# torchmd/torchmd-net

Measured on AMD Instinct MI355X. Metric: molecules/sec (64-atom molecules) TensorNet E+F, higher is better.
Workload: dtype f32; 1 GPU; BASELINE configs[1]: TensorNet F=128 L=2 K=32 rc=5.0, S-mol64 256 molecules x 64 atoms per GPU, energies + forces, random-init weights (seed 0); atoms_per_gpu=16384, pairs_per_gpu=193709, directed_edges_per_gpu=403802, parallelism=molecule-sharded x1, RCCL all-reduce of energies, rank_step=eager: tmdnet_build_graph (pair-count read-back) + tmdnet_energy_forces

## Files before the change

### torchmd-net_amd/csrc/tn_api.hip

```cpp
#include <hip/hip_runtime.h>

#include <algorithm>
#include <cmath>
#include <cstdio>
#include <cstdlib>
#include <cstring>
#include <map>
#include <unordered_map>
#include <string>
#include <vector>

#include "tn_chain.h"
#include "tn_heads.h"
#include "tn_model.h"
#include "tn_tlin9.h"
#include "tn_small.h"
#include "tn_interp.h"
#include "tn_virial.h"

using namespace tn;

static const char* kCatNames[CAT_COUNT] = {"graph", "gemm_edge", "gemm_node", "message", "pair_bwd", "embed_scatter", "elementwise", "edge_table"};

int fail(tmdnet_model* m, int code, const std::string& msg) {
// ... 448 lines not shown
    out.err_slope = worst_s;
    if (getenv("TMDNET_DEBUG"))
      fprintf(stderr, "[tmdnet] radial tables T=%d: value err %.3e, slope err %.3e, fail=%d\n", T, worst_v, worst_s, (int)fail_);
    cleanup(good);
    if (good) {
      out.ok = true;
      out.T = T;
      out.tab = tab;
      for (const TableSpec& sp : specs) out.R.push_back(sp.chain.back().N);
      return TMDNET_OK;
    }
    if (fail_) return TMDNET_OK;
  }
  (void)m;
  return TMDNET_OK;
}

namespace {

int build_edge_tables(tmdnet_model* m) {
  const tmdnet_hparams& hp = m->hp;
  const int F = hp.hidden_channels, K = hp.num_rbf, L = hp.num_layers;
  const DevParams& W = m->P;
  std::vector<TableSpec> specs;
  if (m->tn2) {
    specs.push_back(TableSpec{{TableLayer{W.Wdp, W.bdp, 3 * F, K, 0}}});
    for (int l = 0; l < L; ++l) specs.push_back(TableSpec{{TableLayer{m->tn2->layer[l].M1a, W.layer[l].b1, F, K, 0}}});
  } else if (L + 1 <= 8) {
    specs.push_back(TableSpec{{TableLayer{W.Wdp, W.bdp, 3 * F, K, 0}}});
    for (int l = 0; l < L; ++l) {
      const LayerP& q_ = W.layer[l];
      specs.push_back(TableSpec{{TableLayer{q_.M1, q_.b1, F, K, 1}, TableLayer{q_.M2, q_.b2, 2 * F, F, 1},
                                 TableLayer{q_.M3, q_.b3, 3 * F, 2 * F, 2}}});
    }
  }
  return build_radial_tables(m, m->tabs, specs, W.means, W.betas, K, hp.cutoff_lower, hp.cutoff_upper);
}

}

int ensure_radial_tables(tmdnet_model* m, hipStream_t s) {
  if (!m->tabs_pending) return TMDNET_OK;
  hipStreamCaptureStatus cs = hipStreamCaptureStatusNone;
  if (s && hipStreamIsCapturing(s, &cs) == hipSuccess && cs != hipStreamCaptureStatusNone)
    return fail(m, TMDNET_ERR_STATE, "the radial tables are rebuilt after a parameter upload: run one step outside the capture first");
  HIP_TRY(m, hipDeviceSynchronize());
  const int rc = m->et ? et_build_tables(m) : build_edge_tables(m);
  if (rc != TMDNET_OK) return rc;
  HIP_TRY(m, hipStreamSynchronize(nullptr));
  m->tabs_pending = false;
  return TMDNET_OK;
}

extern "C" {

const char* tmdnet_version(void) { return "tmdnet_amd 0.3 (gfx950)"; }
int tmdnet_abi_version(void) { return TMDNET_ABI_VERSION; }

int tmdnet_create(const tmdnet_hparams* hp, tmdnet_model** out) {
  if (!hp || !out) return TMDNET_ERR_INVALID;
  if (hp->hidden_channels <= 0 || hp->num_layers < 0 || hp->num_rbf <= 0 || hp->max_z <= 0 || hp->head_hidden <= 0 ||
      hp->max_num_neighbors <= 0 || !(hp->cutoff_upper > hp->cutoff_lower))
    return TMDNET_ERR_INVALID;
  tmdnet_model* m = new tmdnet_model();
  m->hp = *hp;
  if (const char* e = getenv("TMDNET_EDGE_TABLE_MIN_PAIRS")) m->tab_min_pairs = atoll(e);
  build_specs(m);
  if (getenv("TMDNET_SIDE_STREAM")) {
    if (hipStreamCreateWithFlags(&m->side, hipStreamNonBlocking) != hipSuccess) m->side = nullptr;
    if (m->side) {
      (void)hipEventCreateWithFlags(&m->ev_fork, hipEventDisableTiming);
      m->ev_join.resize(hp->num_layers);
      for (auto& e : m->ev_join) (void)hipEventCreateWithFlags(&e, hipEventDisableTiming);
    }
  }
  *out = m;
  return TMDNET_OK;
}

int tmdnet_create_tn2(const tmdnet_tn2_hparams* hp, tmdnet_model** out) {
  if (!hp || !out) return TMDNET_ERR_INVALID;
  if (hp->hidden_channels <= 0 || hp->num_layers < 0 || hp->num_rbf <= 0 || hp->max_z <= 0 || hp->head_hidden <= 0 ||
      hp->max_num_neighbors <= 0 || !(hp->cutoff_upper > hp->cutoff_lower) || hp->q_dim <= 0 || hp->q_dim > 64 ||
      (hp->num_layers + 1) * hp->q_dim > 64)
    return TMDNET_ERR_INVALID;
  tmdnet_model* m = new tmdnet_model();
  m->hp = tmdnet_hparams{hp->hidden_channels, hp->num_layers, hp->num_rbf, hp->max_z, hp->max_num_neighbors, hp->group_o3,
                         hp->head_hidden, hp->has_atomref, hp->cutoff_lower, hp->cutoff_upper};
  m->tn2 = new Tn2Model();
  m->tn2->hp = *hp;
  if (const char* e = getenv("TMDNET_EDGE_TABLE_MIN_PAIRS")) m->tab_min_pairs = atoll(e);
  build_specs(m);
  *out = m;
  return TMDNET_OK;
}

int tmdnet_create_et(const tmdnet_et_hparams* hp, tmdnet_model** out) {
  if (!hp || !out) return TMDNET_ERR_INVALID;
  if (hp->hidden_channels <= 0 || hp->num_layers < 0 || hp->num_rbf <= 0 || hp->max_z <= 0 || hp->num_heads <= 0 ||
      hp->max_num_neighbors <= 0 || !(hp->cutoff_upper > hp->cutoff_lower))
    return TMDNET_ERR_INVALID;
  tmdnet_model* m = new tmdnet_model();
  m->hp = tmdnet_hparams{};
  m->hp.hidden_channels = hp->hidden_channels;
  m->hp.num_layers = hp->num_layers;
  m->hp.num_rbf = hp->num_rbf;
  m->hp.max_z = hp->max_z;
  m->hp.max_num_neighbors = hp->max_num_neighbors;
  m->hp.has_atomref = hp->has_atomref;
  m->hp.cutoff_lower = hp->cutoff_lower;
  m->hp.cutoff_upper = hp->cutoff_upper;
  const int rc = et_create(m, hp);
  if (rc != TMDNET_OK) {
    delete m;
    return rc;
  }
  *out = m;
  return TMDNET_OK;
}

int tmdnet_destroy(tmdnet_model* m) {
  if (!m) return TMDNET_OK;
  et_destroy(m);
  if (m->side) {
    (void)hipStreamSynchronize(m->side);
    (void)hipEventDestroy(m->ev_fork);
    for (auto& e : m->ev_join) (void)hipEventDestroy(e);
    (void)hipStreamDestroy(m->side);
  }
  free_radial_tables(m->tabs);
  delete m->tn2;
  if (m->dev) (void)hipFree(m->dev);
  if (m->dev_sb) (void)hipFree(m->dev_sb);
  if (m->upd_tid) (void)hipFree(m->upd_tid);
  if (m->upd_ofs) (void)hipFree(m->upd_ofs);
  if (m->upd_ptrs) (void)hipFree(m->upd_ptrs);
  if (m->rb_img) (void)hipFree(m->rb_img);
  if (m->halo_rng) (void)hipFree(m->halo_rng);
  if (m->prior_tab) (void)hipFree(m->prior_tab);
  delete m;
  return TMDNET_OK;
}

const char* tmdnet_last_error(const tmdnet_model* m) { return m ? m->err.c_str() : "null model"; }

int tmdnet_num_params(const tmdnet_model* m) { return m ? (int)m->specs.size() : 0; }

int tmdnet_set_output_head(tmdnet_model* m, int32_t kind) {
  if (!m) return TMDNET_ERR_INVALID;
  if (kind < TMDNET_HEAD_SCALAR || kind > TMDNET_HEAD_VECTOR)
    return fail(m, TMDNET_ERR_INVALID, "unknown output head kind " + std::to_string(kind));
  if (kind != TMDNET_HEAD_SCALAR && m->tn2)
    return fail(m, TMDNET_ERR_INVALID, "TensorNet2 has the ScalarPlusWeightedCoulomb head only (no property heads)");
  if (kind == TMDNET_HEAD_VECTOR && !m->et)
    return fail(m, TMDNET_ERR_INVALID, "the vector output head needs the Equivariant Transformer's vector features");
  m->host.clear();
  m->finalized = false;
  m->upd_ready = false;
  m->head_kind = kind;
  if (m->et) {
    et_head_specs(m);
    return TMDNET_OK;
  }
  const std::string key = "output_model.atomic_mass";
  auto& sp = m->specs;
  for (size_t i = 0; i < sp.size(); ++i)
    if (sp[i].name == key) {
      sp.erase(sp.begin() + (long)i);
      break;
    }
  if (kind != TMDNET_HEAD_SCALAR) sp.push_back({key, TMDNET_MASS_TABLE_SIZE, 1});
  return TMDNET_OK;
}

const char* tmdnet_param_name(const tmdnet_model* m, int idx, int64_t* numel) {
  if (!m || idx < 0 || idx >= (int)m->specs.size()) return nullptr;
  if (numel) *numel = m->specs[idx].rows * m->specs[idx].cols;
  return m->specs[idx].name.c_str();
}

int tmdnet_set_param(tmdnet_model* m, const char* name, const float* data_host, int64_t numel) {
  if (!m || !name || !data_host) return TMDNET_ERR_INVALID;
  for (const auto& sp : m->specs) {
    if (sp.name == name) {
      if (numel != sp.rows * sp.cols)
        return fail(m, TMDNET_ERR_INVALID, std::string("parameter ") + name + ": expected " + std::to_string(sp.rows * sp.cols) +
                                               " elements, got " + std::to_string(numel));
      m->host[name].assign(data_host, data_host + numel);
      m->finalized = false;
      return TMDNET_OK;
    }
// ... 470 lines not shown
    if (const int rc = ensure_radial_tables(const_cast<tmdnet_model*>(m), nullptr)) return rc;
  if (n == "edge_table_T") *value = m->tabs.ok ? m->tabs.T : 0;
  else if (n == "edge_table_err_value") *value = m->tabs.err_value;
  else if (n == "edge_table_err_slope") *value = m->tabs.err_slope;
  else if (n == "edge_table_min_pairs") *value = (double)m->tab_min_pairs;
  else if (n == "pair_rows_bf16") *value = (double)m->pair_bf16;
  else if (n == "embed_rb_min_atoms") *value = (double)m->rb_min_atoms;
  else if (n == "chain_min_atoms") *value = (double)m->chain_min_atoms;
  else if (n == "chain_mask") *value = (double)m->chain_mask;
  else if (n == "chain_last") *value = (double)m->chain_last;
  else if (n == "recompute_pair_rows") *value = m->recompute_rows ? 1.0 : 0.0;
  else if (n == "embed_rb") *value = m->rb_fwd ? 1.0 : 0.0;
  else if (n == "species_last_build") *value = (double)m->last_nt;
  else if (n == "halo_active_first") *value = (double)m->halo_active[0];
  else if (n == "halo_active_rows") *value = (double)m->halo_active[1];
  else if (n == "message_route_last") *value = (double)m->msg_route_last[0];
  else if (n == "message_adjoint_route_last") *value = (double)m->msg_route_last[1];
  else if (n == "fold_node_adjoint") *value = m->fold_node_adjoint ? 1.0 : 0.0;
  else if (n == "message_adjoint_fold_last") *value = (double)m->msg_fold_last;
  else return TMDNET_ERR_INVALID;
  return TMDNET_OK;
}

int tmdnet_set_cell_grid(tmdnet_model* m, int32_t ncx, int32_t ncy, int32_t ncz) {
  if (!m) return TMDNET_ERR_INVALID;
  if (ncx < 0 || ncy < 0 || ncz < 0) ncx = ncy = ncz = -1;
  m->cell_n[0] = ncx;
  m->cell_n[1] = ncy;
  m->cell_n[2] = ncz;
  return TMDNET_OK;
}

int tmdnet_graph_workspace_bytes(const tmdnet_model* m, int64_t n_atoms, int64_t n_mol, size_t* bytes) {
  if (!m || !bytes || n_atoms < 0 || n_mol < 0) return TMDNET_ERR_INVALID;
  const int64_t ecap = (int64_t)m->hp.max_num_neighbors * n_atoms;
  carve_graph(nullptr, n_atoms, n_mol, ecap, bytes);
  return TMDNET_OK;
}

int tmdnet_build_graph(tmdnet_model* m, void* stream, void* graph_ws, size_t graph_ws_bytes, int64_t n_atoms, int64_t n_mol,
                       const float* pos, const int64_t* batch, const int64_t* z, const float* box, int32_t box_mode,
                       int64_t counts_host[8]) {
  if (!m || !graph_ws || !counts_host || n_atoms < 0 || n_mol < 0) return TMDNET_ERR_INVALID;
  if (n_atoms >= (int64_t)1 << 30) return fail(m, TMDNET_ERR_INVALID, "n_atoms too large for 32-bit indices");
  hipStream_t s = reinterpret_cast<hipStream_t>(stream);
  const int64_t ecap = (int64_t)m->hp.max_num_neighbors * n_atoms;
  size_t need = 0;
  Graph g = carve_graph(graph_ws, n_atoms, n_mol, ecap, &need);
  if (need > graph_ws_bytes) return fail(m, TMDNET_ERR_WORKSPACE, "graph workspace too small");
  if (box_mode != 0 && !box) return fail(m, TMDNET_ERR_INVALID, "box_mode != 0 needs a box");
  const bool cell = cell_applicable(m, n_atoms, n_mol, box_mode);
  set_cell(g, m, cell, n_mol);
  if (cell && m->halo_fn && m->atom_w && !m->et && !m->tn2) g.ghost_w = m->atom_w;
  m->graph_no_ghost_pairs = g.ghost_w != nullptr;
  m->graph_is_cell = cell;
  m->graph_cell_multi = cell && n_mol > 1;
  m->graph_has_z = z != nullptr;
  m->g_pos = pos;
  m->g_box = box;
  m->g_box_mode = box_mode;
  CurScope cur_(m);
  {
    ProfScope ps_(s, CAT_GRAPH, 0.0, (double)n_atoms * 20);
    if (cell) {
      launch_fill(reinterpret_cast<float*>(g.counts), 0.f, 8, s);
      launch_cell_phase1(g, pos, batch, box_mode == 1 ? box : nullptr, (int)n_atoms, m->hp.cutoff_lower, m->hp.cutoff_upper, true, s,
                         (int)n_mol);
      launch_scan_counts(g, (int)n_atoms, s);
    } else {
      launch_graph_build_phase1(g, pos, batch, box, box_mode, (int)n_atoms, (int)n_mol, m->hp.cutoff_lower, m->hp.cutoff_upper,
                                true, s);
    }
    if (z) launch_prepare_z(g, z, cell ? g.perm : nullptr, (int)n_atoms, m->hp.max_z, s);
    if (z && m->rb_fwd && n_atoms >= m->rb_min_atoms) launch_type_map(g, (int)n_atoms, m->hp.max_z, s);
  }
  int counts[8] = {0, 0, 0, 0, 0, 0, 0, 0};
  HIP_TRY(m, hipMemcpyAsync(counts, g.counts, sizeof(counts), hipMemcpyDeviceToHost, s));
  HIP_TRY(m, hipStreamSynchronize(s));
  for (int k = 0; k < 8; ++k) counts_host[k] = counts[k];
  m->last_nt = (z && m->rb_fwd && n_atoms >= m->rb_min_atoms) ? counts[6] : 0;
  m->lastE = counts[1];
  m->graph_closed_tiles = !cell && counts[3] == 0 && counts[5] == 0 && counts[7] == 0;
  remember_graph(m, graph_ws, n_atoms, n_mol);
  if (counts[5])
    return fail(m, TMDNET_ERR_INVALID, "batch index out of range: every entry must be in [0, " + std::to_string(n_mol) + ")");
  if (counts[4])
    return fail(m, TMDNET_ERR_INVALID, "atomic number out of range: every z must be in [0, max_z = " + std::to_string(m->hp.max_z) + ")");
  if (counts[2])
    return fail(m, TMDNET_ERR_OVERFLOW, "Found num_pairs > max_num_pairs, please increase max_num_pairs (found " +
                                            std::to_string(counts[1]) + " edges, capacity " + std::to_string(ecap) + ")");
  m->lastE = counts[1];
  {
    ProfScope ps_(s, CAT_GRAPH, 0.0, (double)counts[1] * 12 + (double)counts[0] * 40);
    if (cell) {
      launch_cell_phase2(g, (int)n_atoms, m->hp.cutoff_lower, m->hp.cutoff_upper, true, s);
      launch_nbr_link_wave(g, (int)n_atoms, s);
    } else {
      launch_graph_build_phase2(g, pos, batch, box, box_mode, (int)n_atoms, (int)n_mol, m->hp.cutoff_lower, m->hp.cutoff_upper, true,
                                s);
    }
  }
  HIP_TRY(m, hipGetLastError());
  return TMDNET_OK;
}

int tmdnet_build_graph_static(tmdnet_model* m, void* stream, void* graph_ws, size_t graph_ws_bytes, int64_t n_atoms, int64_t n_mol,
                              const float* pos, const int64_t* batch, const int64_t* z, const float* box, int32_t box_mode) {
  if (!m || !graph_ws || n_atoms < 0 || n_mol < 0) return TMDNET_ERR_INVALID;
  hipStream_t s = reinterpret_cast<hipStream_t>(stream);
  const int64_t ecap = (int64_t)m->hp.max_num_neighbors * n_atoms;
  size_t need = 0;
  Graph g = carve_graph(graph_ws, n_atoms, n_mol, ecap, &need);
  if (need > graph_ws_bytes) return fail(m, TMDNET_ERR_WORKSPACE, "graph workspace too small");
  if (box_mode != 0 && !box) return fail(m, TMDNET_ERR_INVALID, "box_mode != 0 needs a box");
  const bool cell = cell_applicable(m, n_atoms, n_mol, box_mode);
  set_cell(g, m, cell, n_mol);
  m->graph_no_ghost_pairs = false;
  m->graph_is_cell = cell;
  m->graph_cell_multi = cell && n_mol > 1;
  m->graph_has_z = z != nullptr;
  m->g_pos = pos;
  m->g_box = box;
  m->g_box_mode = box_mode;
  CurScope cur_(m);
  {
    ProfScope ps_(s, CAT_GRAPH, 0.0, (double)n_atoms * 20);
    if (cell) {
      launch_fill(reinterpret_cast<float*>(g.counts), 0.f, 8, s);
      launch_cell_phase1(g, pos, batch, box_mode == 1 ? box : nullptr, (int)n_atoms, m->hp.cutoff_lower, m->hp.cutoff_upper, true, s,
                         (int)n_mol);
      launch_scan_counts(g, (int)n_atoms, s);
      launch_cell_phase2(g, (int)n_atoms, m->hp.cutoff_lower, m->hp.cutoff_upper, true, s);
      launch_nbr_link_wave(g, (int)n_atoms, s);
    } else if (graph_small_ok((int)n_atoms)) {
      launch_graph_small(g, pos, batch, box, box_mode, (int)n_atoms, (int)n_mol, m->hp.cutoff_lower, m->hp.cutoff_upper, true, z,
                         m->hp.max_z, s);
    } else {
      launch_graph_build_phase1(g, pos, batch, box, box_mode, (int)n_atoms, (int)n_mol, m->hp.cutoff_lower, m->hp.cutoff_upper,
                                true, s);
      launch_graph_build_phase2(g, pos, batch, box, box_mode, (int)n_atoms, (int)n_mol, m->hp.cutoff_lower, m->hp.cutoff_upper, true,
                                s);
    }
    if (z && (cell || !graph_small_ok((int)n_atoms))) launch_prepare_z(g, z, cell ? g.perm : nullptr, (int)n_atoms, m->hp.max_z, s);
  }
  m->lastE = ecap;
  m->last_nt = 0;
  m->graph_closed_tiles = false;
  remember_graph(m, graph_ws, n_atoms, n_mol);
  HIP_TRY(m, hipGetLastError());
  return TMDNET_OK;
}

int tmdnet_graph_counts(tmdnet_model* m, void* stream, void* graph_ws, int64_t n_atoms, int64_t n_mol, int64_t counts_host[8]) {
  if (!m || !graph_ws || !counts_host) return TMDNET_ERR_INVALID;
// ... 1154 lines not shown
```

### torchmd-net_amd/csrc/tn_cell.hip

```cpp
#include <cstring>

#include <hip/hip_runtime.h>

#include "tn_common.h"
#include "tn_kernels.h"

namespace tn {

static inline int cdivc(int64_t a, int64_t b) { return (int)((a + b - 1) / b); }

size_t cell_sort_temp_bytes(int64_t n) { return (size_t)(8 * (n > 0 ? n : 1) + 2) * sizeof(int); }

__global__ void k_cell_assign(const float* __restrict__ pos, const float* __restrict__ box, int N, const int* __restrict__ cgrid,
                              int* __restrict__ key, int* __restrict__ hist) {
  int i = blockIdx.x * blockDim.x + threadIdx.x;
  if (i >= N) return;
  const int ncx = cgrid[0], ncy = cgrid[1], ncz = cgrid[2];
  const float x = pos[i * 3], y = pos[i * 3 + 1], zc = pos[i * 3 + 2];
  float fz = zc / box[8];
  float fy = (y - fz * box[7]) / box[4];
  float fx = (x - fy * box[3] - fz * box[6]) / box[0];
  fx -= floorf(fx);
  fy -= floorf(fy);
  fz -= floorf(fz);
// ... 71 lines not shown
__global__ void k_permute_pos(const float* __restrict__ pos, const int64_t* __restrict__ batch, const int* __restrict__ perm, int N,
                              int B, float* __restrict__ pos_s, int* __restrict__ bat_s, int64_t* __restrict__ bat_c,
                              int* __restrict__ counts) {
  int i = blockIdx.x * blockDim.x + threadIdx.x;
  if (i >= N) return;
  const int o = perm[i];
  pos_s[i * 3] = pos[o * 3];
  pos_s[i * 3 + 1] = pos[o * 3 + 1];
  pos_s[i * 3 + 2] = pos[o * 3 + 2];
  if (batch) {
    int64_t b = batch[o];
    if (B > 0 && (b < 0 || b >= B)) {
      counts[5] = 1;
      b = b < 0 ? 0 : B - 1;
    }
    bat_s[i] = (int)b;
    bat_c[i] = b;
    if (i == 0) counts[3] = 1;
  }
}
__global__ void k_permute_z(const int64_t* __restrict__ z, const int* __restrict__ perm, int N, int64_t* __restrict__ z_s) {
  int i = blockIdx.x * blockDim.x + threadIdx.x;
  if (i < N) z_s[i] = z[perm[i]];
}
void launch_permute_z(const Graph& g, const int64_t* z, int N, hipStream_t s) {
  hipLaunchKernelGGL(k_permute_z, dim3(cdivc(N, 256)), dim3(256), 0, s, z, g.perm, N, g.z_s);
}
__global__ void k_prepare_z(const int64_t* __restrict__ z, const int* __restrict__ perm, int N, int max_z, int64_t* __restrict__ z_c,
                            int* __restrict__ counts) {
  int i = blockIdx.x * blockDim.x + threadIdx.x;
  if (i >= N) return;
  int64_t v = z[perm ? perm[i] : i];
  if (v < 0 || v >= max_z) {
    counts[4] = 1;
    v = v < 0 ? 0 : max_z - 1;
  }
  z_c[i] = v;
}
void launch_prepare_z(const Graph& g, const int64_t* z, const int* perm, int N, int max_z, hipStream_t s) {
  if (N <= 0) return;
  hipLaunchKernelGGL(k_prepare_z, dim3(cdivc(N, 256)), dim3(256), 0, s, z, perm, N, max_z, g.z_c, g.counts);
}

__device__ __forceinline__ float cell_d2(const float* __restrict__ pos, int hi, int lo, const float* __restrict__ box, float& dx,
                                         float& dy, float& dz) {
  return pair_geometry(pos, hi, lo, box, dx, dy, dz);
}

template <bool FILL>
__global__ __launch_bounds__(256) void k_nbr_cell(Graph g, int N, float lo2, float up2, int loop) {
  const int i = blockIdx.x * 4 + (threadIdx.x >> 6);
  const int lane = threadIdx.x & 63;
  if (i >= N) return;
  if (FILL && g.counts[2]) return;
  const float* __restrict__ pos = g.pos_s;
  const float* __restrict__ box = g.boxd;
  const int* __restrict__ bat = g.use_cell > 1 ? g.bat_s : nullptr;
  const int ncx = g.cgrid[0], ncy = g.cgrid[1], ncz = g.cgrid[2];
  const int ci = g.cell_key_sorted[i];
  const int bi = bat ? bat[i] : 0;
  const float* __restrict__ gw = g.ghost_w;
  const bool ghost_i = gw && gw[g.perm[i]] == 0.f;
  const int cz = ci % ncz, cy = (ci / ncz) % ncy, cx = ci / (ncz * ncy);
  int nid = 0x7fffffff;
  if (lane < 27) {
    const int dx = lane / 9 - 1, dy = (lane / 3) % 3 - 1, dz = lane % 3 - 1;
    const int x = (cx + dx + ncx) % ncx, y = (cy + dy + ncy) % ncy, zc = (cz + dz + ncz) % ncz;
    nid = (x * ncy + y) * ncz + zc;
  }
#pragma unroll
  for (int k = 2; k <= 32; k <<= 1)
#pragma unroll
    for (int j = k >> 1; j > 0; j >>= 1) {
      const int other = __shfl_xor(nid, j, 64);
      const bool up = ((lane & k) == 0);
      const bool lower = ((lane & j) == 0);
      nid = (lower == up) ? min(nid, other) : max(nid, other);
    }
  const int P = FILL ? g.counts[0] : 0;
  int e = FILL ? g.rowptr[i] : 0, p = FILL ? g.pairptr[i] : 0;
  int nl = 0, nt = 0;
  const unsigned long long lt = lane == 0 ? 0ull : (~0ull >> (64 - lane));
  int t = 0;
  while (t < 27) {
    int c0 = __shfl(nid, t, 64), c1 = c0;
    ++t;
    while (t < 27) {
      const int cn = __shfl(nid, t, 64);
      if (cn != c1 && cn != c1 + 1) break;
      c1 = cn;
      ++t;
    }
    const int j0 = g.cell_start[c0], j1 = g.cell_start[c1 + 1];
    for (int base = j0; base < j1; base += 64) {
      const int j = base + lane;
      bool hit = false, self = false;
      float dx = 0.f, dy = 0.f, dz = 0.f, d2 = 0.f;
      if (j < j1) {
        if (j == i) {
          hit = loop != 0;
          self = true;
        } else if ((!bat || bat[j] == bi) && !(ghost_i && gw[g.perm[j]] == 0.f)) {
          d2 = (j < i) ? cell_d2(pos, i, j, box, dx, dy, dz) : cell_d2(pos, j, i, box, dx, dy, dz);
          hit = d2 < up2 && d2 >= lo2;
        }
      }
      const unsigned long long mall = __ballot(hit);
// ... 127 lines not shown
```

### torchmd-net_amd/csrc/tn_graph_wave.hip

```cpp
#include <cstdlib>

#include "tn_common.h"
#include "tn_kernels.h"

namespace tn {

static inline int cdivw(int64_t a, int64_t b) { return (int)((a + b - 1) / b); }

__device__ __forceinline__ float pair_d2(const float* __restrict__ pos, int hi, int lo, const float* __restrict__ box, float& dx,
                                         float& dy, float& dz) {
  return pair_geometry(pos, hi, lo, box, dx, dy, dz);
}

template <bool FILL>
__device__ __forceinline__ void nbr_wave_row(const Graph& g, const float* __restrict__ pos, const int64_t* __restrict__ batch,
                                             const float* __restrict__ box, int box_mode, int N, int B, float lo2, float up2, int loop,
                                             int i, int lane) {
  int64_t b = batch[i];
  int j0 = 0, j1 = N;
  if (b < 0 || b >= B) {
    b = 0;
    j1 = 0;
  } else if (!g.counts[3]) {
    j0 = g.mstart[b];
// ... 13 lines not shown
        hit = loop != 0;
        self = true;
      } else if (batch[j] == b) {
        d2 = (j < i) ? pair_d2(pos, i, j, bx, dx, dy, dz) : pair_d2(pos, j, i, bx, dx, dy, dz);
        hit = d2 < up2 && d2 >= lo2;
      }
    }
    const unsigned long long mall = __ballot(hit);
    const unsigned long long mlow = __ballot(hit && j < i);
    if (FILL) {
      if (hit) {
        const int ee = e + __popcll(mall & lt);
        g.col[ee] = j;
        if (self) {
          g.epair[ee] = P;
          g.esign[ee] = 0.f;
        } else if (j < i) {
          const int pp = p + __popcll(mlow & lt);
          const float d = sqrtf(d2);
          const float inv = d > 0.f ? 1.0f / d : 0.f;
          g.pair_i[pp] = i;
          g.pair_j[pp] = j;
          g.pd[pp] = d;
          g.pdelta[pp * 3 + 0] = dx; g.pdelta[pp * 3 + 1] = dy; g.pdelta[pp * 3 + 2] = dz;
          g.prhat[pp * 3 + 0] = dx * inv; g.prhat[pp * 3 + 1] = dy * inv; g.prhat[pp * 3 + 2] = dz * inv;
          g.epair[ee] = pp;
          g.esign[ee] = 1.f;
        } else {
          g.epair[ee] = -1;
          g.esign[ee] = -1.f;
        }
      }
      e += __popcll(mall);
      p += __popcll(mlow);
    } else {
      nt += __popcll(mall);
      nl += __popcll(mlow);
    }
  }
  if (!FILL && lane == 0) {
    g.nlow[i] = nl;
    g.ntot[i] = nt;
  }
  if (FILL && i == 0 && lane == 0) g.pd[P] = 0.f;
}

template <bool FILL>
__global__ __launch_bounds__(256) void k_nbr_wave(Graph g, const float* __restrict__ pos, const int64_t* __restrict__ batch,
                                                  const float* __restrict__ box, int box_mode, int N, int B, float lo2, float up2,
                                                  int loop) {
  const int i = blockIdx.x * 4 + (threadIdx.x >> 6);
  const int lane = threadIdx.x & 63;
  if (i >= N) return;
  if (FILL && g.counts[2]) return;
  nbr_wave_row<FILL>(g, pos, batch, box, box_mode, N, B, lo2, up2, loop, i, lane);
}

__device__ __forceinline__ void nbr_link_row(const Graph& g, int i, int lane) {
  const int e0 = g.rowptr[i], e1 = g.rowptr[i + 1];
  for (int e = e0 + lane; e < e1; e += 64) {
    const int j = g.col[e];
    if (j <= i) continue;
    int lo = g.rowptr[j], hi = lo + g.nlow[j] - 1;
    const int base = lo;
    while (lo < hi) {
      const int mid = (lo + hi) >> 1;
      if (g.col[mid] < i) lo = mid + 1; else hi = mid;
    }
    g.epair[e] = g.pairptr[j] + (lo - base);
  }
}
__global__ __launch_bounds__(256) void k_nbr_link_wave(Graph g, int N) {
  const int i = blockIdx.x * 4 + (threadIdx.x >> 6);
  const int lane = threadIdx.x & 63;
  if (i >= N || g.counts[2]) return;
  nbr_link_row(g, i, lane);
}

constexpr int GS_MAX_ATOMS = 256;
constexpr int GS_ECAP = 16384;
__global__ __launch_bounds__(1024) void k_graph_small(Graph g, const float* __restrict__ pos, const int64_t* __restrict__ batch,
                                                      const float* __restrict__ box, int box_mode, int N, int B, float lo2, float up2,
                                                      int loop, const int64_t* __restrict__ z, int max_z) {
  __shared__ int s_mstart[GS_MAX_ATOMS], s_mend[GS_MAX_ATOMS], s_nlow[GS_MAX_ATOMS], s_ntot[GS_MAX_ATOMS];
  __shared__ int s_rowptr[GS_MAX_ATOMS + 1], s_pairptr[GS_MAX_ATOMS + 1], s_counts[8], c_low[4], c_tot[4];
  __shared__ float s_pos[3 * GS_MAX_ATOMS];
  __shared__ int64_t s_batch[GS_MAX_ATOMS];
  __shared__ int s_col[GS_ECAP];
  const bool col_lds = g.ecap <= GS_ECAP;
  const int tid = threadIdx.x, lane = tid & 63, wave = tid >> 6;
  const bool mol_lds = B <= GS_MAX_ATOMS;
  Graph gl = g;
  gl.nlow = s_nlow;
  gl.ntot = s_ntot;
  gl.rowptr = s_rowptr;
  gl.pairptr = s_pairptr;
  gl.counts = s_counts;
  if (mol_lds) {
    gl.mstart = s_mstart;
    gl.mend = s_mend;
  }
  if (col_lds) gl.col = s_col;
  for (int k = tid; k < 3 * N; k += 1024) s_pos[k] = pos[k];
  if (tid < N) s_batch[tid] = batch[tid];
  for (int i = tid; i < B; i += 1024) gl.mstart[i] = gl.mend[i] = 0;
  if (tid < 8) s_counts[tid] = 0;
  __syncthreads();
  if (tid < N) {
    const int i = tid;
    const int64_t b = s_batch[i];
    if (b < 0 || b >= B) {
      s_counts[3] = 1;
      s_counts[5] = 1;
    } else {
      if (i > 0) {
        const int64_t bp = s_batch[i - 1];
        if (bp > b) s_counts[3] = 1;
        if (bp != b) gl.mstart[b] = i;
        else if ((i & 63) == 0) s_counts[7] = 1;
      } else {
        gl.mstart[b] = 0;
      }
      if (i == N - 1 || s_batch[i + 1] != b) gl.mend[b] = i + 1;
    }
    if (z) {
      int64_t v = z[i];
      if (v < 0 || v >= max_z) {
        s_counts[4] = 1;
// ... 97 lines not shown
```

### torchmd-net_amd/csrc/tn_kernels.h

```cpp
#pragma once
#include <hip/hip_runtime.h>
#include <stdint.h>

namespace tn {

struct Graph {
  int* mstart;
  int* mend;
  int* nlow;
  int* ntot;
  int* rowptr;
  int* pairptr;
  int* col;
  int* epair;
  float* esign;
  int* pair_i;
  int* pair_j;
  float* pd;
  float* pdelta;
  float* prhat;
  int* counts;
  int* tix;
  int* tz;
  int64_t ecap, pcap;
  int* perm;
  int* iota;
  int* cell_key;
  int* cell_key_sorted;
  int* cell_start;
  float* pos_s;
  int64_t* z_s;
  float* boxd;
  int* cgrid;
  int* bat_s;
  int64_t* bat_c;
  int64_t* z_c;
  void* sort_tmp;
  size_t sort_tmp_bytes;
  int ncx, ncy, ncz;
  int use_cell;
  const float* ghost_w;
  int max_z;
  int small_mols;
};

struct RadialParams {
  const float* means;
  const float* betas;
  int K;
  float lo, up;
};

void launch_graph_build_phase1(const Graph& g, const float* pos, const int64_t* batch, const float* box, int box_mode, int N,
                               int B, float lo, float up, bool loop, hipStream_t s);
void launch_graph_build_phase2(const Graph& g, const float* pos, const int64_t* batch, const float* box, int box_mode, int N,
                               int B, float lo, float up, bool loop, hipStream_t s);
void launch_export_pairs(const Graph& g, int N, bool include_transpose, bool loop, int64_t max_pairs, const int* perm,
                         int64_t* neighbors, float* deltas, float* distances, int* num_pairs, hipStream_t s);

void launch_neighbor_grad(const int64_t* nb, const float* deltas, const float* dist, const float* g_delta, const float* g_dist,
                          int64_t M, int N, float* out, hipStream_t s);

void launch_radial(const Graph& g, int P, RadialParams rp, float* phi, float* dphi, float* C, float* dC, hipStream_t s);

void launch_ztables(const float* emb, const float* WaT, const float* WbT, const float* b2, int Z, int F, float* Utab, float* Vtab,
                    hipStream_t s);
void launch_embed_scatter(const Graph& g, int N, int F, const int64_t* z, const float* Utab, const float* Vtab, const float* Q,
                          const float* C, float* u0, float* s0n, hipStream_t s);
void launch_layernorm_fwd(const float* x, const float* w, const float* b, int rows, int R, float* y, float* xhat, float* rstd,
                          hipStream_t s);
void launch_layernorm_bwd(const float* g, const float* xhat, const float* rstd, const float* w, int rows, int R, float* gx,
                          hipStream_t s);
void launch_norm_x(const float* X, float* Xh, int N, int F, hipStream_t s);
struct PairRowTable;
enum MsgRoute {
  MSG_NONE = 0,
  MSG_FWD_ROW = 1,
  MSG_FWD_SPLIT = 2,
  MSG_FWD_TILE = 3,
  MSG_ADJ_ROW = 4,
  MSG_ADJ_SPLIT = 5,
  MSG_GD_ROW = 6,
  MSG_GD_SPLIT = 7,
  MSG_GD_TILE = 8,
  MSG_DUAL = 9,
  MSG_DUAL_ACC = 10,
  MSG_FWD_ROW_TABLE = 11,
  MSG_FWD_ROW_RANGE = 12,
  MSG_GD_ROW_TABLE = 13,
  MSG_GD_ROW_OWNED = 14,
  MSG_GD_ROW_TWO = 15,
  MSG_DUAL_SPLIT3 = 16,
};
MsgRoute message_route(const Graph& g, int N, int F, bool rows_from_table = false, int row0 = 0, int nrows = -1);
MsgRoute message_adjoint_route(int N, int F);
MsgRoute message_adjoint_gd_route(const Graph& g, int N, int F, bool rows_from_table = false, int own0 = 0, int own1 = -1,
// ... 127 lines not shown
```

### torchmd-net_amd/csrc/tn_kernels.hip

```cpp
#include "tn_kernels.h"
#include "tn_interp.h"

#include <cstdlib>

#include "tn_common.h"

namespace tn {

static inline int fthreads(int F) {
  int t = ((F + 63) / 64) * 64;
  return t > 256 ? 256 : t;
}
static inline int cdiv(int64_t a, int64_t b) { return (int)((a + b - 1) / b); }

__global__ void k_mol_ranges(const int64_t* __restrict__ batch, int N, int B, int* mstart, int* mend, int* counts) {
  int i = blockIdx.x * blockDim.x + threadIdx.x;
  if (i >= N) return;
  int64_t b = batch[i];
  if (b < 0 || b >= B) {
    counts[3] = 1;
    counts[5] = 1;
    return;
  }
  if (i > 0) {
// ... 78 lines not shown
    for (int off = 1; off < 64; off <<= 1) {
      int ta = __shfl_up(ia, off, 64), tb = __shfl_up(ib, off, 64);
      if (lane >= off) {
        ia += ta;
        ib += tb;
      }
    }
    if (lane == 63) {
      wsum[0][wave] = ia;
      wsum[1][wave] = ib;
    }
    __syncthreads();
    int oa = carry[0] + ia - a, ob = carry[1] + ib - b;
    for (int w = 0; w < wave; ++w) {
      oa += wsum[0][w];
      ob += wsum[1][w];
    }
#pragma unroll
    for (int r = 0; r < PER; ++r) {
      la[tid * PER + r] = oa;
      lb[tid * PER + r] = ob;
      oa += va[r];
      ob += vb[r];
    }
    __syncthreads();
    if (tid == 1023) {
      carry[0] = oa;
      carry[1] = ob;
    }
#pragma unroll
    for (int r = 0; r < PER; ++r) {
      const int i = base + r * 1024 + tid;
      if (i < N) {
        g.pairptr[i] = la[r * 1024 + tid];
        g.rowptr[i] = lb[r * 1024 + tid];
      }
    }
    __syncthreads();
  }
  if (tid == 0) {
    const int P = carry[0], E = carry[1];
    g.pairptr[N] = P;
    g.rowptr[N] = E;
    g.counts[0] = P;
    g.counts[1] = E;
    g.counts[2] = (E > g.ecap || P > g.pcap || g.counts[5]) ? 1 : 0;
  }
}

__global__ void k_nbr_fill(Graph g, const float* __restrict__ pos, const int64_t* __restrict__ batch, const float* __restrict__ box,
                           int box_mode, int N, float lo2, float up2, int loop) {
  int i = blockIdx.x * blockDim.x + threadIdx.x;
  if (i >= N) return;
  if (g.counts[2]) return;
  const int P = g.counts[0];
  int64_t b = batch[i];
  int j0, j1;
  cand_range(g.mstart, g.mend, g.counts, b, N, j0, j1);
  const float* bx = box_mode == 0 ? nullptr : (box_mode == 1 ? box : box + b * 9);
  int e = g.rowptr[i];
  int p = g.pairptr[i];
  for (int j = j0; j < j1; ++j) {
    if (j == i) {
      if (loop) {
        g.col[e] = i;
        g.epair[e] = P;
        g.esign[e] = 0.f;
        ++e;
      }
      continue;
    }
    if (batch[j] != b) continue;
    float dx, dy, dz;
    float d2 = (j < i) ? pair_delta(pos, i, j, bx, dx, dy, dz) : pair_delta(pos, j, i, bx, dx, dy, dz);
    if (d2 < up2 && d2 >= lo2) {
      g.col[e] = j;
      if (j < i) {
        float d = sqrtf(d2);
        float inv = d > 0.f ? 1.0f / d : 0.f;
        g.pair_i[p] = i;
        g.pair_j[p] = j;
        g.pd[p] = d;
        g.pdelta[p * 3 + 0] = dx;
        g.pdelta[p * 3 + 1] = dy;
        g.pdelta[p * 3 + 2] = dz;
        g.prhat[p * 3 + 0] = dx * inv;
        g.prhat[p * 3 + 1] = dy * inv;
        g.prhat[p * 3 + 2] = dz * inv;
        g.epair[e] = p;
        g.esign[e] = 1.f;
        ++p;
      } else {
        g.epair[e] = -1;
        g.esign[e] = -1.f;
      }
      ++e;
    }
  }
  if (i == 0) g.pd[P] = 0.f;
}

__global__ void k_nbr_link(Graph g, int N) {
  int i = blockIdx.x * blockDim.x + threadIdx.x;
  if (i >= N) return;
  if (g.counts[2]) return;
  int e0 = g.rowptr[i], e1 = g.rowptr[i + 1];
  for (int e = e0; e < e1; ++e) {
    int j = g.col[e];
    if (j <= i) continue;
    int lo = g.rowptr[j], hi = lo + g.nlow[j] - 1, base = lo;
    while (lo < hi) {
      int mid = (lo + hi) >> 1;
      if (g.col[mid] < i) lo = mid + 1; else hi = mid;
    }
    g.epair[e] = g.pairptr[j] + (lo - base);
  }
}

__global__ void k_graph_reset(Graph g, int B) {
  const int i = blockIdx.x * blockDim.x + threadIdx.x;
  if (i < B) g.mstart[i] = g.mend[i] = 0;
  if (i < 8) g.counts[i] = 0;
}

void launch_graph_build_phase1(const Graph& g, const float* pos, const int64_t* batch, const float* box, int box_mode, int N,
                               int B, float lo, float up, bool loop, hipStream_t s) {
  hipLaunchKernelGGL(k_graph_reset, dim3(cdiv(B > 8 ? B : 8, 256)), dim3(256), 0, s, g, B);
  if (N <= 0) return;
  hipLaunchKernelGGL(k_mol_ranges, dim3(cdiv(N, 256)), dim3(256), 0, s, batch, N, B, g.mstart, g.mend, g.counts);
  if (getenv("TMDNET_SCALAR_GRAPH"))
    hipLaunchKernelGGL(k_nbr_count, dim3(cdiv(N, 64)), dim3(64), 0, s, g, pos, batch, box, box_mode, N, lo * lo, up * up, (int)loop);
  else
    launch_nbr_count_wave(g, pos, batch, box, box_mode, N, B, lo, up, loop, s);
  hipLaunchKernelGGL(k_scan_counts, dim3(1), dim3(1024), 0, s, g, N);
}

void launch_scan_counts(const Graph& g, int N, hipStream_t s) {
  hipLaunchKernelGGL(k_scan_counts, dim3(1), dim3(1024), 0, s, g, N);
}

void launch_graph_build_phase2(const Graph& g, const float* pos, const int64_t* batch, const float* box, int box_mode, int N,
                               int B, float lo, float up, bool loop, hipStream_t s) {
  if (N <= 0) return;
  if (getenv("TMDNET_SCALAR_GRAPH")) {
    hipLaunchKernelGGL(k_nbr_fill, dim3(cdiv(N, 64)), dim3(64), 0, s, g, pos, batch, box, box_mode, N, lo * lo, up * up, (int)loop);
    hipLaunchKernelGGL(k_nbr_link, dim3(cdiv(N, 64)), dim3(64), 0, s, g, N);
  } else {
    launch_nbr_fill_link_wave(g, pos, batch, box, box_mode, N, B, lo, up, loop, s);
  }
}

__global__ void k_export_pairs(Graph g, int N, int include_transpose, int loop, int64_t max_pairs, const int* __restrict__ perm,
                               int64_t* neighbors, float* deltas, float* distances, int* num_pairs) {
  const int P = g.counts[0];
  const int64_t total = (int64_t)P * (include_transpose ? 2 : 1) + (loop ? N : 0);
  int64_t idx = (int64_t)blockIdx.x * blockDim.x + threadIdx.x;
  if (idx == 0) num_pairs[0] = (int)total;
  if (idx >= max_pairs) return;
// ... 1319 lines not shown
```

### torchmd-net_amd/csrc/tn_model.h

```cpp
#pragma once
#include <hip/hip_runtime.h>

#include <cstdio>
#include <cstring>
#include <map>
#include <string>
#include <unordered_map>
#include <vector>

#include "../../include/tmdnet_amd.h"
#include "tn_gemm.h"
#include "tn_kernels.h"
#include "tn_prior_math.h"
#include "tn_train.h"

using namespace tn;


struct LayerP {
  const float *M1, *b1, *M2, *b2, *M3, *b3;
  const float *M2T, *M3T;
  const float* V[6];
  const float* VT[6];
  const uint16_t* M_sb[3];
// ... 89 lines not shown
  std::vector<Tn2LayerP> layer;
  const float* qweights = nullptr;
};

struct EdgeTables {
  bool ok = false;
  int T = 0;
  std::vector<float*> tab;
  std::vector<int> R;
  double err_value = 0.0, err_slope = 0.0;
};
struct TableLayer {
  const float* W;
  const float* b;
  int N, K, kind;
};
struct TableSpec {
  std::vector<TableLayer> chain;
};

struct TrainCtx {
  int phase = 0;
  const float* gE = nullptr;
  float* grads = nullptr;
  std::map<std::string, int64_t> off;
  std::vector<float*> pre1, he1, pre2, he2, pre3, Ch, Xh;
  float *g3 = nullptr, *g2 = nullptr, *g1 = nullptr;
  float *self_gw = nullptr, *gq = nullptr, *selfq = nullptr, *gZu = nullptr, *gZv = nullptr, *onehot = nullptr, *head = nullptr;
  float *part = nullptr, *wT = nullptr, *forces = nullptr;
  float* at(const std::string& k) const { return grads + off.at(k); }
};

struct tmdnet_model {
  bool recompute_rows = false;
  const float* atom_w = nullptr;
  int (*halo_fn)(void*, int32_t, float*, int64_t, int64_t, const int32_t*, void*) = nullptr;
  void* halo_user = nullptr;
  int* halo_rng = nullptr;
  bool graph_no_ghost_pairs = false;
  int halo_active[2] = {0, 0};
  bool fold_node_adjoint = true;
  bool graph_closed_tiles = false;
  int msg_fold_last = 0;
  int msg_route_last[2] = {0, 0};
  tmdnet_hparams hp;
  int head_kind = 0;
  TrainCtx* train = nullptr;
  float* virial_out = nullptr;
  void* virial_ws = nullptr;
  std::vector<std::pair<std::string, int64_t>> train_entries;
  hipStream_t side = nullptr;
  hipEvent_t ev_fork = nullptr;
  std::vector<hipEvent_t> ev_join;
  EtModel* et = nullptr;
  Tn2Model* tn2 = nullptr;
  const float* g_pos = nullptr;
  const float* g_box = nullptr;
  int g_box_mode = 0;
  Profiler prof;
  int64_t lastE = 0;
  int cell_n[3] = {0, 0, 0};
  bool graph_is_cell = false;
  bool graph_cell_multi = false;
  bool graph_has_z = false;
  struct GraphRecord { bool is_cell, cell_multi, has_z; int nt; int64_t lastE; bool no_ghost_pairs; int64_t n_atoms, n_mol; bool closed_tiles; };
  std::unordered_map<const void*, GraphRecord> graph_rec;
  std::vector<ParamSpec> specs;
  std::map<std::string, std::vector<float>> host;
  float* dev = nullptr;
  size_t dev_cap = 0, dev_sb_cap = 0, rb_cap = 0;
  uint16_t* dev_sb = nullptr;
  std::unordered_map<const float*, const uint16_t*> sb_of;
  std::unordered_map<const float*, const uint16_t*> fm_of;
  struct ImageJob { size_t src_off; int64_t n, k; size_t dst_off; int fm; };
  std::vector<ImageJob> image_jobs;
  size_t packed_elems = 0;
  int32_t* upd_tid = nullptr;
  int32_t* upd_ofs = nullptr;
  const float** upd_ptrs = nullptr;
  bool upd_ready = false;
  DevParams P;
  EdgeTables tabs;
  uint16_t* rb_img = nullptr;
  const uint16_t *rb_fwd = nullptr, *rb_rev = nullptr;
  int last_nt = 0;
  int64_t rb_min_atoms = 1024;
  int64_t chain_min_atoms = 4096;
  int chain_mask = 7;
  int chain_last = 0;
  int pair_bf16 = 0;
  bool tabs_pending = false;
  int64_t tab_min_pairs = 1;
  bool finalized = false;
  std::string err;
  FwdBuffers last{};
  int64_t lastN = 0, lastP = 0;
  bool has_last = false;
  const float* tn2_last_chg = nullptr;
  int prior_flags = 0, prior_max_z = 0;
  float* prior_tab = nullptr;
  size_t prior_cap = 0;
  tn_prior::ZblConst prior_zbl{};
  tn_prior::D2Const prior_d2{};
};


// ... 97 lines not shown
```

Before: 116,500 molecules/s.

## Overlap graph phase-2 build with pinned pair-count read-back

The pair counts are now read back into a pinned host buffer with an event, and the phase-2 neighbour fill/link kernels are queued before the host waits, so the copy and the host sync overlap with the GPU's fill work instead of leaving the device idle. Because phase 2 now runs before the host checks overflow, the kernels gain a device-side guard (refuse_z with counts[4]) so they skip writing when an error flag is set. This removes a host round-trip bubble per step. The risk is that error handling now depends on device-side flags rather than host checks made before launch.

Result: no change. 117,500 molecules/s (median of 6 runs) (+0.9%).

```diff
diff --git a/torchmd-net_amd/csrc/tn_api.hip b/torchmd-net_amd/csrc/tn_api.hip
--- a/torchmd-net_amd/csrc/tn_api.hip
+++ b/torchmd-net_amd/csrc/tn_api.hip
@@ -524,6 +524,27 @@
   return TMDNET_OK;
 }
 
+static int ensure_counts_readback(tmdnet_model* m) {
+  if (!m->counts_pin) {
+    void* p = nullptr;
+    if (hipHostMalloc(&p, 8 * sizeof(int), hipHostMallocDefault) != hipSuccess) {
+      (void)hipGetLastError();
+      return fail(m, TMDNET_ERR_HIP, "hipHostMalloc of the graph counts' read-back buffer failed");
+    }
+    m->counts_pin = static_cast<int*>(p);
+  }
+  if (!m->ev_counts && hipEventCreateWithFlags(&m->ev_counts, hipEventDisableTiming) != hipSuccess) {
+    (void)hipGetLastError();
+    m->ev_counts = nullptr;
+    return fail(m, TMDNET_ERR_HIP, "hipEventCreate of the graph counts' read-back event failed");
+  }
+  return TMDNET_OK;
+}
+static void create_counts_readback(tmdnet_model* m) {
+  (void)ensure_counts_readback(m);
+  m->err.clear();
+}
+
 extern "C" {
 
 const char* tmdnet_version(void) { return "tmdnet_amd 0.3 (gfx950)"; }
@@ -546,6 +567,7 @@
       for (auto& e : m->ev_join) (void)hipEventCreateWithFlags(&e, hipEventDisableTiming);
     }
   }
+  create_counts_readback(m);
   *out = m;
   return TMDNET_OK;
 }
@@ -563,6 +585,7 @@
   m->tn2->hp = *hp;
   if (const char* e = getenv("TMDNET_EDGE_TABLE_MIN_PAIRS")) m->tab_min_pairs = atoll(e);
   build_specs(m);
+  create_counts_readback(m);
   *out = m;
   return TMDNET_OK;
 }
@@ -587,6 +610,7 @@
     delete m;
     return rc;
   }
+  create_counts_readback(m);
   *out = m;
   return TMDNET_OK;
 }
@@ -609,6 +633,8 @@
   if (m->upd_ptrs) (void)hipFree(m->upd_ptrs);
   if (m->rb_img) (void)hipFree(m->rb_img);
   if (m->halo_rng) (void)hipFree(m->halo_rng);
+  if (m->ev_counts) (void)hipEventDestroy(m->ev_counts);
+  if (m->counts_pin) (void)hipHostFree(m->counts_pin);
   if (m->prior_tab) (void)hipFree(m->prior_tab);
   delete m;
   return TMDNET_OK;
@@ -1185,6 +1211,7 @@
   const bool cell = cell_applicable(m, n_atoms, n_mol, box_mode);
   set_cell(g, m, cell, n_mol);
   if (cell && m->halo_fn && m->atom_w && !m->et && !m->tn2) g.ghost_w = m->atom_w;
+  g.refuse_z = 1;
   m->graph_no_ghost_pairs = g.ghost_w != nullptr;
   m->graph_is_cell = cell;
   m->graph_cell_multi = cell && n_mol > 1;
@@ -1207,10 +1234,24 @@
     if (z) launch_prepare_z(g, z, cell ? g.perm : nullptr, (int)n_atoms, m->hp.max_z, s);
     if (z && m->rb_fwd && n_atoms >= m->rb_min_atoms) launch_type_map(g, (int)n_atoms, m->hp.max_z, s);
   }
-  int counts[8] = {0, 0, 0, 0, 0, 0, 0, 0};
-  HIP_TRY(m, hipMemcpyAsync(counts, g.counts, sizeof(counts), hipMemcpyDeviceToHost, s));
-  HIP_TRY(m, hipStreamSynchronize(s));
-  for (int k = 0; k < 8; ++k) counts_host[k] = counts[k];
+  if (const int rc = ensure_counts_readback(m)) return rc;
+  HIP_TRY(m, hipMemcpyAsync(m->counts_pin, g.counts, 8 * sizeof(int), hipMemcpyDeviceToHost, s));
+  HIP_TRY(m, hipEventRecord(m->ev_counts, s));
+  int ps2 = -1;
+  {
+    ProfScope ps_(s, CAT_GRAPH, 0.0, 0.0);
+    ps2 = ps_.idx;
+    if (cell) {
+      launch_cell_phase2(g, (int)n_atoms, m->hp.cutoff_lower, m->hp.cutoff_upper, true, s);
+      launch_nbr_link_wave(g, (int)n_atoms, s);
+    } else {
+      launch_graph_build_phase2(g, pos, batch, box, box_mode, (int)n_atoms, (int)n_mol, m->hp.cutoff_lower, m->hp.cutoff_upper, true,
+                                s);
+    }
+  }
+  HIP_TRY(m, hipEventSynchronize(m->ev_counts));
+  int counts[8];
+  for (int k = 0; k < 8; ++k) counts_host[k] = counts[k] = m->counts_pin[k];
   m->last_nt = (z && m->rb_fwd && n_atoms >= m->rb_min_atoms) ? counts[6] : 0;
   m->lastE = counts[1];
   m->graph_closed_tiles = !cell && counts[3] == 0 && counts[5] == 0 && counts[7] == 0;
@@ -1223,16 +1264,7 @@
     return fail(m, TMDNET_ERR_OVERFLOW, "Found num_pairs > max_num_pairs, please increase max_num_pairs (found " +
                                             std::to_string(counts[1]) + " edges, capacity " + std::to_string(ecap) + ")");
   m->lastE = counts[1];
-  {
-    ProfScope ps_(s, CAT_GRAPH, 0.0, (double)counts[1] * 12 + (double)counts[0] * 40);
-    if (cell) {
-      launch_cell_phase2(g, (int)n_atoms, m->hp.cutoff_lower, m->hp.cutoff_upper, true, s);
-      launch_nbr_link_wave(g, (int)n_atoms, s);
-    } else {
-      launch_graph_build_phase2(g, pos, batch, box, box_mode, (int)n_atoms, (int)n_mol, m->hp.cutoff_lower, m->hp.cutoff_upper, true,
-                                s);
-    }
-  }
+  if (ps2 >= 0) m->prof.recs[ps2].bytes = (double)counts[1] * 12 + (double)counts[0] * 40;
   HIP_TRY(m, hipGetLastError());
   return TMDNET_OK;
 }
diff --git a/torchmd-net_amd/csrc/tn_cell.hip b/torchmd-net_amd/csrc/tn_cell.hip
--- a/torchmd-net_amd/csrc/tn_cell.hip
+++ b/torchmd-net_amd/csrc/tn_cell.hip
@@ -147,7 +147,7 @@
   const int i = blockIdx.x * 4 + (threadIdx.x >> 6);
   const int lane = threadIdx.x & 63;
   if (i >= N) return;
-  if (FILL && g.counts[2]) return;
+  if (FILL && (g.counts[2] || (g.refuse_z && g.counts[4]))) return;
   const float* __restrict__ pos = g.pos_s;
   const float* __restrict__ box = g.boxd;
   const int* __restrict__ bat = g.use_cell > 1 ? g.bat_s : nullptr;
diff --git a/torchmd-net_amd/csrc/tn_graph_wave.hip b/torchmd-net_amd/csrc/tn_graph_wave.hip
--- a/torchmd-net_amd/csrc/tn_graph_wave.hip
+++ b/torchmd-net_amd/csrc/tn_graph_wave.hip
@@ -89,7 +89,7 @@
   const int i = blockIdx.x * 4 + (threadIdx.x >> 6);
   const int lane = threadIdx.x & 63;
   if (i >= N) return;
-  if (FILL && g.counts[2]) return;
+  if (FILL && (g.counts[2] || (g.refuse_z && g.counts[4]))) return;
   nbr_wave_row<FILL>(g, pos, batch, box, box_mode, N, B, lo2, up2, loop, i, lane);
 }
 
@@ -110,7 +110,7 @@
 __global__ __launch_bounds__(256) void k_nbr_link_wave(Graph g, int N) {
   const int i = blockIdx.x * 4 + (threadIdx.x >> 6);
   const int lane = threadIdx.x & 63;
-  if (i >= N || g.counts[2]) return;
+  if (i >= N || (g.counts[2] || (g.refuse_z && g.counts[4]))) return;
   nbr_link_row(g, i, lane);
 }
 
diff --git a/torchmd-net_amd/csrc/tn_kernels.h b/torchmd-net_amd/csrc/tn_kernels.h
--- a/torchmd-net_amd/csrc/tn_kernels.h
+++ b/torchmd-net_amd/csrc/tn_kernels.h
@@ -42,6 +42,7 @@
   const float* ghost_w;
   int max_z;
   int small_mols;
+  int refuse_z;
 };
 
 struct RadialParams {
diff --git a/torchmd-net_amd/csrc/tn_kernels.hip b/torchmd-net_amd/csrc/tn_kernels.hip
--- a/torchmd-net_amd/csrc/tn_kernels.hip
+++ b/torchmd-net_amd/csrc/tn_kernels.hip
@@ -154,7 +154,7 @@
                            int box_mode, int N, float lo2, float up2, int loop) {
   int i = blockIdx.x * blockDim.x + threadIdx.x;
   if (i >= N) return;
-  if (g.counts[2]) return;
+  if (g.counts[2] || (g.refuse_z && g.counts[4])) return;
   const int P = g.counts[0];
   int64_t b = batch[i];
   int j0, j1;
@@ -205,7 +205,7 @@
 __global__ void k_nbr_link(Graph g, int N) {
   int i = blockIdx.x * blockDim.x + threadIdx.x;
   if (i >= N) return;
-  if (g.counts[2]) return;
+  if (g.counts[2] || (g.refuse_z && g.counts[4])) return;
   int e0 = g.rowptr[i], e1 = g.rowptr[i + 1];
   for (int e = e0; e < e1; ++e) {
     int j = g.col[e];
diff --git a/torchmd-net_amd/csrc/tn_model.h b/torchmd-net_amd/csrc/tn_model.h
--- a/torchmd-net_amd/csrc/tn_model.h
+++ b/torchmd-net_amd/csrc/tn_model.h
@@ -165,6 +165,8 @@
   hipStream_t side = nullptr;
   hipEvent_t ev_fork = nullptr;
   std::vector<hipEvent_t> ev_join;
+  int* counts_pin = nullptr;
+  hipEvent_t ev_counts = nullptr;
   EtModel* et = nullptr;
   Tn2Model* tn2 = nullptr;
   const float* g_pos = nullptr;
```
